# olsonanl/signature_kmers

Measured on AMD Instinct MI355X. Metric: k-mers/sec (extract+hash+count) at 1/2/4/8 GPUs; achieved HBM GB/s %, higher is better.
Workload: dtype u8

## Files before the change

### signature_kmers_amd/__init__.py

```python
from __future__ import annotations

import ctypes as C
import os
from dataclasses import dataclass

import numpy as np

__all__ = [
    "SkmError", "lib", "K", "UNDEFINED_FUNCTION", "STORED_DTYPE", "CALL_DTYPE",
    "SignatureBuilder", "KeptKmers", "CmphKmerDb", "FunctionCaller", "mph_build",
    "kmer_to_str", "str_to_kmer", "keys_from_strings", "device_count", "MatrixDistance", "SeqIdMap",
    "matrix_tile_rows",
]

K = 8
UNDEFINED_FUNCTION = 0xFFFF
_HERE = os.path.dirname(os.path.abspath(__file__))
LIB_PATH = os.environ.get("SKM_LIB_PATH") or os.path.join(_HERE, "libskm.so")

STORED_DTYPE = np.dtype([("avg_from_end", "<u2"), ("function_index", "<u2"), ("mean", "<u2"),
                         ("median", "<u2"), ("var", "<u2")])
CALL_DTYPE = np.dtype([("start", "<u4"), ("end", "<u4"), ("count", "<i4"), ("function_index", "<u2"),
                       ("pad", "<u2"), ("protein_length_median", "<u4"),
                       ("protein_length_med_avg_dev", "<f4")])
# ... 269 lines not shown
            return {}
        ms = (C.c_float * n)()
        cnt = (C.c_uint64 * n)()
        buf = C.create_string_buffer(64 * n + 64)
        lib().skm_build_kernel_timings(self._h, buf, len(buf), ms, cnt, n)
        names = buf.value.decode().split("\n")[:n]
        return {names[i]: (float(ms[i]), int(cnt[i])) for i in range(n)}

    def set_option(self, name: str, value: int):
        _check(lib().skm_build_set_option(self._h, name.encode(), int(value)))

    def passes(self) -> int:
        return self.counters()["passes"]

    def counters(self) -> dict:
        v = (C.c_uint64 * 46)()
        n = lib().skm_build_counters(self._h, v, 46)
        names = ["windows", "kept", "overflow_subbuckets", "chain_jobs", "chain_samples", "sequences", "grouped",
                 "overflow_elements", "overflow_kept", "big_groups", "big_kept", "passes", "valid", "giant_chains",
                 "giant_max", "redone", "cap_overflow_scratch", "cap_split", "cap_long_samples", "cap_long_jobs",
                 "demand_overflow_scratch", "demand_split", "demand_long_samples", "demand_long_jobs",
                 "long_samples", "routed", "add_batch_us", "prepare_upload_us", "prepare_plan_us", "prepare_rest_us",
                 "pass_groups", "add_pack_us", "add_dma_wait_us", "finish_us", "finish_wait_us", "finish_copy_us",
                 "finish_chunks", "finish_select_dev_us", "finish_sort_dev_us", "finish_gather_dev_us",
                 "finish_d2h_dev_us", "finish_max_chunk", "finish_wide_index", "kept_cap",
                 "free_after_prepare", "recs_rot"]
        return {names[i]: int(v[i]) for i in range(n)}

    def debug_jobs(self, k: int = 64) -> list:
        v = (C.c_uint32 * k)()
        _check(lib().skm_build_debug_jobs(self._h, v, k))
        return [int(x) for x in v]

    def debug_overflow(self, k: int = 4096) -> list:
        v = (C.c_uint32 * k)()
        n = lib().skm_build_debug_overflow(self._h, v, k)
        return [int(x) for x in v[:min(max(n, 0), k)]]

    def debug_stamps(self, enable: bool) -> list:
        v = (C.c_uint64 * 32)()
        _check(lib().skm_build_debug_stamps(self._h, 1 if enable else 0, v, 32))
# ... 465 lines not shown
```

### signature_kmers_amd/csrc/skm_build.hip

```cpp
#include <hip/hip_runtime.h>

#include <algorithm>
#include <type_traits>
#include <chrono>
#include <cmath>
#include <cstdio>
#include <cstdlib>
#include <cstring>
#include <deque>
#include <functional>
#include <memory>
#include <numeric>
#include <string>
#include <thread>
#include <vector>

#include "skm_common.h"
#include "skm_pool.h"
#include "skm_output.h"
#include "skm_util.h"

#if defined(SKM_WITH_RCCL)
#include <rccl/rccl.h>
#endif
// ... 616 lines not shown
    return true;
}

enum : uint32_t {
    RUN_FLAGS = 0,
    RUN_LONG_CUR = 1,
    RUN_LONG_N = 2,
    RUN_LONG_FLUSHED = 3,
    RUN_SNAP = 28,
    RUN_DEM_TOT = 8,
    RUN_DEM_SPLIT = 9,
    RUN_DEM_LONG = 10,
    RUN_DEM_LJOBS = 11,
    RUN_LONG_WANT = 12,
    RUN_LONG_WANTJ = 13,
    RUN_ACC_NOVF = 16,
    RUN_ACC_JOBS = 17,
    RUN_ACC_LENS = 18,
    RUN_ACC_OVF_ELEMS = 19,
    RUN_ACC_OVF_KEPT = 20,
    RUN_ACC_BIG = 21,
    RUN_ACC_BIG_KEPT = 22,
    RUN_ACC_GROUPED = 23,
    RUN_LAST_NOVF = 24,
    RUN_LAST_JOBS = 25,
    RUN_NLOC = 26,
    RUN_SLOTS = 64
};
constexpr unsigned long long RUN_F_ARENA = 1;
constexpr unsigned long long RUN_F_RERUN = 2;
constexpr unsigned long long RUN_F_CAP = 4;
enum : uint32_t {
    PLAN_NOVF = 0,
    PLAN_NSPLIT = 1,
    PLAN_NHEAVY = 2,
    PLAN_SKIP = 3,
    PLAN_Q_SPLIT = 4,
    PLAN_Q_HEAVY = 5,
    PLAN_Q_REST = 6,
    PLAN_SLOTS = 8
};

constexpr int JOB_CLASSES = 32;
constexpr int JOB_WG = 256;

__device__ __forceinline__ uint32_t job_class(uint32_t n) { return 31u - (uint32_t)__clz(n | 1u); }

__device__ __forceinline__ void job_chunk(const unsigned long long* nj_p, uint64_t cap, uint64_t& a, uint64_t& e) {
    const uint64_t nj = min((uint64_t)*nj_p, cap);
    const uint64_t chunk = (nj + gridDim.x - 1) / gridDim.x;
    a = min(nj, (uint64_t)blockIdx.x * chunk);
    e = min(nj, a + chunk);
}

// ... 1533 lines not shown
    uint32_t nbuckets;
    uint32_t bucket_base;
    int rem_bits;
    const uint32_t* glen;
    uint8_t* flags;
    unsigned long long* ctr;
    uint64_t* out_keys;
    skm_stored_kmer_data* out_data;
    Job* jobs;
    uint32_t* lens;
    OvfEntry* ovf;
    uint32_t ovf_cap;
    unsigned long long* stamps;
    uint64_t* big_desc;
    uint32_t big_cap;
    int prio;
    int pshift;
    int flag_check;
    const uint32_t* skip;
    uint32_t sub_target;
    int diag;
    const uint32_t* order;
    int part_class;
};

#define SKM_STAMP(i)                                                          \
    do {                                                                      \
        if (A.stamps && threadIdx.x == 0) {                                   \
            const uint64_t _t = __builtin_amdgcn_s_memtime();                 \
            atomicAdd(&A.stamps[(i)], (unsigned long long)(_t - *L.tlast));   \
// ... 186 lines not shown

constexpr uint32_t LPER = CAP / BPK_THREADS;

__device__ __forceinline__ void load_batch(const uint64_t* __restrict__ src_hi, const uint64_t* __restrict__ src_lo,
                                           uint32_t n, uint64_t (&eh)[LPER], uint64_t (&el)[LPER]) {
#pragma unroll
    for (uint32_t u = 0; u < LPER; ++u) {
        const uint32_t j = threadIdx.x + u * BPK_THREADS;
        if (j < n) {
            eh[u] = __builtin_nontemporal_load(src_hi + j);
            el[u] = __builtin_nontemporal_load(src_lo + j);
        }
    }
}

__device__ __forceinline__ void process_sub(const uint64_t* __restrict__ src_hi, const uint64_t* __restrict__ src_lo,
                                            uint32_t n, const BucketArgs& A, uint64_t hprefix, const SubLds& L) {
    const uint32_t tid = threadIdx.x, nt = blockDim.x;
    const uint32_t EMPTY = 0xFFFFFFFFu;
    uint64_t eh[LPER], el[LPER];
    load_batch(src_hi, src_lo, n, eh, el);
    for (uint32_t t = tid; t < (uint32_t)TAB; t += nt) L.tab[t] = EMPTY;
#pragma unroll
    for (uint32_t u = 0; u < LPER; ++u) {
        const uint32_t j = tid + u * BPK_THREADS;
        if (j < n) {
            L.hi[j] = eh[u];
            L.lo[j] = el[u];
        }
    }
    if (tid == 0) *L.nbig = 0;
// ... 78 lines not shown
    if (tid == 0) {
        uint32_t run = 0, acc = 0;
        for (int q = 0; q < 7; ++q) {
            const uint32_t t = ccnt[q];
            ccnt[q] = run;
            cstart[q] = run;
            tstart[q] = acc;
            const uint32_t per = q < 6 ? (64u >> (q + 1)) : 1u;
            acc += (t + per - 1) / per;
            run += t;
        }
        cstart[7] = run;
        tstart[7] = acc;
    }
    unsigned long long big_base = 0;
    if (tid == 0 && cstart[7] > cstart[6]) big_base = atomicAdd(&A.ctr[5], (unsigned long long)(cstart[7] - cstart[6]));
    __syncthreads();
    for (uint32_t g = tid; g < G; g += nt) {
        const uint32_t a = L.goff[L.glist[g]];
        const uint32_t c = g + 1 < G ? L.goff[L.glist[g + 1]] - a : M - a;
        L.big[atomicAdd(&ccnt[cls_of(c)], 1u)] = (uint16_t)g;
    }
    if (tid == 0) *reinterpret_cast<unsigned long long*>(L.wave + 44) = big_base;
    __syncthreads();
    SKM_STAMP(6);
    {
        const uint32_t ntask = tstart[6];
        const uint32_t nbig = cstart[7] - cstart[6];
        const uint64_t bbase = *reinterpret_cast<const unsigned long long*>(L.wave + 44);
        const uint32_t wave = tid >> 6, nwaves = nt >> 6, lane = tid & 63u;
        uint64_t* slots = reinterpret_cast<uint64_t*>(L.lens32);
// ... 91 lines not shown
        }
        const uint64_t jbase = njob ? s_base[1] : 0;
#pragma unroll 1
        for (uint32_t t = tid; t < njob; t += nt) {
            const uint32_t j = L.order[t];
            const uint32_t jb = jobinfo[j];
            Job jbr;
            jbr.lens_off = L.lens_sel + 2 * (jb >> 16);
            jbr.n = jb & JOB_COUNT_MASK;
            jbr.out_idx = (uint32_t)(ob + L.rank[j]);
            A.jobs[jbase + t] = jbr;
        }
    }
    __syncthreads();
    SKM_STAMP(8);
}

__global__ __launch_bounds__(BPK_THREADS, BPK_WAVES_EU) void k_bucket_process(BucketArgs A) {
    static_assert(CAP % BPK_THREADS == 0, "emit assigns CAP / BPK_THREADS elements per thread");
    __shared__ uint64_t s_hi[CAP];
    __shared__ uint64_t s_lo[CAP];
    __shared__ uint32_t s_tab[TAB];
    __shared__ uint32_t s_sub[(1 << MAX_B2) + 1];
    __align__(16) __shared__ uint16_t s_slot[CAP];
    __align__(16) __shared__ uint16_t s_rank[CAP];
    __align__(16) __shared__ uint16_t s_goff[CAP];
    __align__(16) __shared__ uint16_t s_glist[CAP];
    __align__(16) __shared__ uint16_t s_order[CAP];
    __align__(16) __shared__ uint16_t s_big[CAP / 2];
    __shared__ __align__(16) uint32_t s_wave[48];
    __shared__ uint32_t s_nbig;
    __shared__ uint64_t s_tlast;
    __shared__ uint32_t s_ccnt[24];
    if (A.skip && *A.skip) return;
    SubLds L;
    L.ccnt = s_ccnt;
    L.tlast = &s_tlast;
    if (threadIdx.x == 0) s_tlast = __builtin_amdgcn_s_memtime();
    L.hi = s_hi;
    L.lo = s_lo;
    L.tab = s_tab;
    L.slot = s_slot;
    L.rank = s_rank;
    L.goff = s_goff;
    L.glist = s_glist;
    L.order = s_order;
    L.big = s_big;
    L.wave = s_wave;
    L.nbig = &s_nbig;

    const uint32_t bucket = blockIdx.x;
    if (bucket >= A.nbuckets) return;
    const uint64_t r0 = A.bstart[bucket], r1 = A.bstart[bucket + 1];
    const uint64_t n = r1 - r0;
    if (n == 0) return;
    const uint64_t hprefix = (uint64_t)(A.bucket_base + bucket) << A.rem_bits;
    if (A.prio == 1) __builtin_amdgcn_s_setprio(1);
    if (A.prio == 2) __builtin_amdgcn_s_setprio(2);
    if (A.prio >= 3) __builtin_amdgcn_s_setprio(3);

    const bool direct = n <= (uint64_t)CAP && A.nsrc == 1;
    uint32_t nsub = 1;
    if (!direct) {
        const uint32_t* tab = A.sub_tab + (uint64_t)bucket * SUB_TAB;
// ... 472 lines not shown
__global__ __launch_bounds__(BP_THREADS) void k_overflow(BucketArgs A, OvfScratch S, uint32_t* plan, int lo_slot,
                                                          int hi_slot, int q_slot, uint32_t inline_min, int prio) {
    __shared__ uint64_t s_hi[CAP];
    __shared__ uint64_t s_lo[CAP];
    __shared__ __align__(16) uint32_t s_wave[48];
    __shared__ uint32_t s_nbig;
    __shared__ uint32_t s_big[BP_THREADS];
    __shared__ uint32_t s_ninl;
    __shared__ uint64_t s_inl[OVF_INLINE_CAP][2];
    __shared__ uint32_t s_q;
    const uint32_t q_lo = lo_slot < 0 ? 0u : plan[lo_slot], q_hi = plan[hi_slot];
    auto entry = [&](const OvfEntry e) {
        if (e.n == 0) return;
        if ((A.diag & 32) && e.n <= (uint32_t)CAP) return;
        if ((A.diag & 64) && e.n > (uint32_t)CAP) return;
        const uint64_t* src_hi = (e.src == 2 ? S.hi : e.src ? A.tmp_hi : A.recs_hi) + e.off;
        const uint64_t* src_lo = (e.src == 2 ? S.lo : e.src ? A.tmp_lo : A.recs_lo) + e.off;
        uint64_t* ghi = S.hi + e.scratch;
        uint64_t* glo = S.lo + e.scratch;
        uint32_t* heads = S.heads + e.scratch;
        uint64_t* jobinfo = S.jobinfo + e.scratch;
        uint32_t* fmean = S.fmean + e.scratch;
        const uint32_t n = e.n;
        uint32_t N = CAP;
        while (N < n) N <<= 1;
        const uint32_t tid = threadIdx.x, nt = blockDim.x;
        const uint64_t hprefix = (uint64_t)(A.bucket_base + e.bucket) << A.rem_bits;
        const uint32_t nch = (n + CAP - 1) / CAP * CAP;
        for (uint32_t c0 = nch; c0 < N; c0 += CAP)
            for (uint32_t j = tid; j < CAP; j += nt) {
                ghi[c0 + j] = ~0ull;
                glo[c0 + j] = ~0ull;
// ... 216 lines not shown
        }
        __syncthreads();
        const uint32_t q = s_q;
        if (q >= q_hi) break;
        entry(A.ovf[q]);
        __syncthreads();
    }
}

constexpr uint32_t HEAVY_MIN = 1024;
constexpr uint32_t SPLIT_MIN = CAP + 1;
constexpr uint32_t SPLIT_TAB = 4096;
constexpr uint32_t SPLIT_MAXH = 256;
constexpr uint32_t HEAVY_WG = 512;
constexpr uint32_t HEAVY_GRID = 1024;

struct HeavyKey {
    uint64_t off;
    uint32_t n;
    uint32_t bucket;
    uint32_t rem;
    uint32_t pad;
};

struct HeavyArgs {
    HeavyKey* keys;
    unsigned long long* nkeys;
    unsigned long long* cursor;
    unsigned long long* queue;
    uint64_t* rec;
// ... 10 lines not shown
    uint64_t gcap;
    unsigned long long* gstat;
};

__device__ __forceinline__ uint32_t split_hash(uint32_t rem) { return (rem * 0x9E3779B1u) >> (32 - 12); }

__device__ __forceinline__ uint64_t heavy_rec(uint64_t hi, uint64_t lo) {
    return (lo & ~((1ull << 36) - 1ull)) | ((lo & 0xFFFFull) << 16) | (hi & 0xFFFFull);
}
__device__ __forceinline__ uint32_t hr_func(uint64_t x) { return (uint32_t)x & 0xFFFFu; }
__device__ __forceinline__ uint32_t hr_off(uint64_t x) { return (uint32_t)(x >> 16) & 0xFFFFu; }
__device__ __forceinline__ uint32_t hr_seq(uint64_t x) { return (uint32_t)(x >> 36); }

constexpr uint32_t SPLIT_U = 8;

__global__ __launch_bounds__(BP_THREADS) void k_ovf_split(BucketArgs A, OvfScratch S, HeavyArgs H, uint32_t heavy_min,
                                                           uint32_t* plan) {
    static_assert(SPLIT_TAB == 4096, "split_hash yields 12 bits");
    __shared__ uint32_t s_key[SPLIT_TAB];
    __shared__ uint32_t s_cnt[SPLIT_TAB];
    __shared__ uint16_t s_hid[SPLIT_TAB];
    __shared__ uint64_t s_hbase[SPLIT_MAXH];
    __shared__ uint32_t s_hcur[SPLIT_MAXH];
    __shared__ uint32_t s_nh, s_fail, s_lcur, s_heavy;
    const uint32_t tid = threadIdx.x, nt = blockDim.x, lane = tid & 63u;
    __shared__ uint32_t s_q;
    const uint32_t q_hi = plan[PLAN_NSPLIT];
    auto entry = [&](const uint32_t qe) {
        OvfEntry e = A.ovf[qe];
        const uint64_t* src_hi = (e.src ? A.tmp_hi : A.recs_hi) + e.off;
        const uint64_t* src_lo = (e.src ? A.tmp_lo : A.recs_lo) + e.off;
// ... 55 lines not shown
                    const uint64_t hk = atomicAdd(H.nkeys, 1ull);
                    const uint64_t base = atomicAdd(H.cursor, (unsigned long long)s_cnt[q]);
                    s_hbase[h] = base;
                    HeavyKey K;
                    K.off = base;
                    K.n = s_cnt[q];
                    K.bucket = e.bucket;
                    K.rem = s_key[q];
                    K.pad = 0;
                    H.keys[hk] = K;
                    atomicAdd(&s_heavy, s_cnt[q]);
                }
            }
        __syncthreads();
        if (s_heavy == 0) return;
        uint64_t* lhi = S.hi + e.scratch;
        uint64_t* llo = S.lo + e.scratch;
        for (uint32_t j0 = 0; j0 < n; j0 += nt * SPLIT_U) {
            uint64_t eh[SPLIT_U], el[SPLIT_U];
    #pragma unroll
            for (uint32_t u = 0; u < SPLIT_U; ++u) {
                const uint32_t j = j0 + u * nt + tid;
                eh[u] = j < n ? src_hi[j] : ~0ull;
                el[u] = j < n ? src_lo[j] : 0ull;
            }
    #pragma unroll
            for (uint32_t u = 0; u < SPLIT_U; ++u) {
                const bool v = eh[u] != ~0ull;
                uint32_t hid = 0xFFFFu;
                if (v) {
                    const uint32_t rem = (uint32_t)(eh[u] >> 16) & REM_MASK;
                    uint32_t slot = split_hash(rem);
                    while (s_key[slot] != rem) slot = (slot + 1) & (SPLIT_TAB - 1);
                    hid = s_hid[slot];
                }
                const uint64_t lm = __ballot(v && hid == 0xFFFFu);
                uint32_t lbase = 0;
                if (lm) {
                    const uint32_t leader = (uint32_t)(__ffsll((long long)lm) - 1);
                    if (lane == leader) lbase = atomicAdd(&s_lcur, (uint32_t)__popcll(lm));
                    lbase = (uint32_t)__shfl((int)lbase, (int)leader, 64);
                }
                if (v && hid == 0xFFFFu) {
                    const uint32_t pos = lbase + (uint32_t)__popcll(lm & lt);
                    lhi[pos] = eh[u];
                    llo[pos] = el[u];
                }
                const uint32_t h0 = (uint32_t)__builtin_amdgcn_readfirstlane((int)(v ? hid : 0xFFFFu));
                const uint64_t hm = __ballot(v && hid != 0xFFFFu && hid == h0);
                uint32_t hbase = 0;
// ... 1 lines not shown
                    const uint32_t leader = (uint32_t)(__ffsll((long long)hm) - 1);
                    if (lane == leader) hbase = atomicAdd(&s_hcur[h0], (uint32_t)__popcll(hm));
                    hbase = (uint32_t)__shfl((int)hbase, (int)leader, 64);
                }
                if (v && hid != 0xFFFFu) {
                    const uint32_t pos = hid == h0 ? hbase + (uint32_t)__popcll(hm & lt) : atomicAdd(&s_hcur[hid], 1u);
                    const uint64_t o = s_hbase[hid] + pos;
                    H.rec[o] = heavy_rec(eh[u], el[u]);
                    H.len[o] = elem_len(eh[u], el[u], A.glen);
                }
            }
        }
        __syncthreads();
        if (tid == 0) {
            e.n = n - s_heavy;
            e.src = 2;
            e.off = e.scratch;
            A.ovf[qe] = e;
        }
    };
    for (;;) {
        if (tid == 0) s_q = atomicAdd(&plan[PLAN_Q_SPLIT], 1u);
        __syncthreads();
        const uint32_t q = s_q;
        if (q >= q_hi) break;
        entry(q);
        __syncthreads();
    }
}

constexpr int RB = 9;
constexpr uint32_t RBINS = 1u << RB;
__device__ uint32_t* wg_radix_sort_u32(uint32_t* a, uint32_t* b, uint32_t n, int bits, uint32_t* s_hist,
                                       uint32_t (*s_wc)[RBINS], uint32_t* s_run, uint32_t& tag) {
    const uint32_t tid = threadIdx.x, nt = blockDim.x, lane = tid & 63u, wave = tid >> 6, nw = nt >> 6;
    const uint64_t lt = (1ull << lane) - 1ull;
    for (int shift = 0; shift < bits; shift += RB) {
        for (uint32_t d = tid; d < RBINS; d += nt) s_hist[d] = 0;
        __syncthreads();
        for (uint32_t j0 = 0; j0 < n; j0 += nt * SPLIT_U) {
            uint32_t x[SPLIT_U];
#pragma unroll
// ... 585 lines not shown
        const uint64_t tot = s_tot, split = s_split, nl = *P.nloc;
        atomicMax(&R[RUN_DEM_TOT], (unsigned long long)tot);
        atomicMax(&R[RUN_DEM_SPLIT], (unsigned long long)split);
        if (raw > P.ovf_cap) atomicOr(&R[RUN_FLAGS], RUN_F_CAP);
        const bool over = tot > P.tot_cap || split > P.split_cap;
        if (over) atomicOr(&R[RUN_FLAGS], RUN_F_RERUN);
        if (P.kept[0] + nl > P.kept_cap) atomicOr(&R[RUN_FLAGS], RUN_F_ARENA);
        const bool skip = over || (atomicAdd(&R[RUN_FLAGS], 0ull) & (RUN_F_ARENA | RUN_F_CAP)) != 0;
        P.plan[PLAN_NOVF] = skip ? 0u : n;
        P.plan[PLAN_NSPLIT] = skip ? 0u : s_nsplit;
        P.plan[PLAN_NHEAVY] = skip ? 0u : s_nheavy;
        P.plan[PLAN_SKIP] = skip ? 1u : 0u;
        P.plan[PLAN_Q_SPLIT] = 0;
        P.plan[PLAN_Q_HEAVY] = 0;
        P.plan[PLAN_Q_REST] = 0;
        R[RUN_ACC_NOVF] += n;
        R[RUN_ACC_OVF_ELEMS] += s_elems;
        R[RUN_ACC_GROUPED] += nl;
        R[RUN_LAST_NOVF] = n;
    }
}

__global__ void k_poison_jobs(Job* __restrict__ jobs, uint64_t n, uint64_t samples, uint32_t idx,
                             skm_stored_kmer_data* __restrict__ out) {
    const uint64_t t = (uint64_t)blockIdx.x * blockDim.x + threadIdx.x;
    for (uint64_t j = t; j < n; j += (uint64_t)gridDim.x * blockDim.x) jobs[j] = Job{samples, 8u, idx};
    if (t == 0) out[idx] = skm_stored_kmer_data{0xC0DE, 0xC0DE, 0xC0DE, 0xC0DE, 0xC0DE};
}

__global__ void k_pass_account(const unsigned long long* __restrict__ ctr, unsigned long long* __restrict__ run,
                               uint64_t jobs_cap, uint64_t jobs2_cap, uint64_t big_cap, uint64_t lens_cap) {
    const unsigned long long j = ctr[3] + ctr[8 + 3];
    run[RUN_ACC_JOBS] += j;
    run[RUN_ACC_LENS] += ctr[8 + 4];
    run[RUN_ACC_OVF_KEPT] += ctr[8];
    run[RUN_ACC_BIG] += ctr[5];
    run[RUN_ACC_BIG_KEPT] += ctr[6];
    run[RUN_LAST_JOBS] = j;
    if (ctr[3] > jobs_cap || ctr[8 + 3] > jobs2_cap || ctr[5] > big_cap || ctr[8 + 4] > lens_cap)
        atomicOr(&run[RUN_FLAGS], RUN_F_CAP);
}

__global__ void k_kept_finalize(uint64_t* __restrict__ keys, const skm_stored_kmer_data* __restrict__ data,
                                const unsigned long long* __restrict__ n_p, uint32_t nf, uint32_t* __restrict__ dfunc) {
    extern __shared__ uint32_t s_h[];
    const uint64_t n = *n_p;
    const bool lds = nf <= 16384;
    if (lds)
        for (uint32_t f = threadIdx.x; f < nf; f += blockDim.x) s_h[f] = 0;
    __syncthreads();
    for (uint64_t i = (uint64_t)blockIdx.x * blockDim.x + threadIdx.x; i < n; i += (uint64_t)gridDim.x * blockDim.x) {
        keys[i] = decode_key(unmix43(keys[i]));
// ... 126 lines not shown
struct Tune {
    int passes = 0;
    int64_t mem_budget_mb = 0;
    int ovf_heavy = 8192;
    int ovf_inline_min = 0x7FFFFFFF;
    int inline_prio = 3;
    int ovf_long_class = 14;
    int main_long_class = 14;
    int ovf_chain_wgs = 0;
    int chain_prio = 0;
    int bucket_prio = 0;
    int chain_lds_kb = 0;
    int host_timing = 0;
    int heavy_min = (int)HEAVY_MIN;
    int split_min = (int)SPLIT_MIN;
    int giant_class = -1;
    int giant_passes = 0;
    int prefetch = 1;
    int heavy_grid = (int)HEAVY_GRID;
    int ovf_grid = 1024;
    int split_grid = 512;
    int chain_grid = 4096;
    int stream_prio = 0;
    int chain_batches = 2;
    int chain_streams = 1;
    int poison_jobs = 0;
    int route_vacate = 0;
    int tail_async = 1;
    int big_grid = 2048;
    int big_grid_large = 512;
// ... 34 lines not shown
    DevBuf hist, offs, sorted, long_off;
};

struct skm_build {
    skm_build_opts opts{};
    int device = 0;
    hipStream_t stream = nullptr;
    struct EvSet {
        hipEvent_t ev[13] = {}, o[3] = {}, o3[3] = {};
    };
    std::deque<EvSet> evsets;
    hipEvent_t* ev = nullptr;
    hipEvent_t* ev_o = nullptr;
    hipEvent_t* ev_o3 = nullptr;
    float last_ms[15] = {};
    uint64_t ovf_elems = 0, ovf_kept = 0;

    uint8_t* st_pin[2] = {};
    size_t st_fill[2] = {};
    hipEvent_t st_ev[2] = {};
    bool st_busy[2] = {};
    int st_cur = 0;
    uint64_t rp_total = 0;
    uint64_t rp_dev = 0;
    uint64_t res_cap = 0;
    std::vector<SeqMeta> h_meta;
    std::vector<uint32_t> h_seqid;
    std::unique_ptr<HostPool> pool;
    HandoffStats handoff;
    std::vector<uint32_t> h_keep;
    std::vector<uint64_t> h_cum;
// ... 42 lines not shown
#if defined(SKM_WITH_RCCL)
    ncclComm_t comm = nullptr;
#endif
    std::vector<skm_build*> group;
    skm_transport tp{};

    hipStream_t stream2 = nullptr, stream3 = nullptr;
    hipStream_t stream_tail = nullptr;
    hipStream_t stream_tail2 = nullptr;
    hipEvent_t ev_tail_bp = nullptr, ev_tail_done = nullptr, ev_tail2 = nullptr;
    bool tail_pending = false;
    std::function<void()> tail_issue;
    hipEvent_t ev_scan = nullptr;
    bool rot = false;
    uint64_t free_after_prepare = 0;
    hipEvent_t ev_part = nullptr, ev_split = nullptr, ev_part_heavy = nullptr;
    DevBuf d_hv_keys, d_hv_rec, d_hv_len, d_hv_s0, d_hv_s1;
    DevBuf d_sub_tab, d_jobs2, d_jobs3;

    unsigned long long* h_pin = nullptr;
    OvfEntry* h_ovf = nullptr;
    size_t h_ovf_cap = 0;
    unsigned long long* pinned_ctr() {
        if (!h_pin) SKM_HIP(hipHostMalloc(reinterpret_cast<void**>(&h_pin), 128 * 8, hipHostMallocDefault));
        return h_pin;
    }
    OvfEntry* pinned_ovf(size_t n) {
        if (n > h_ovf_cap) {
            if (h_ovf) SKM_HIP(hipHostFree(h_ovf));
            h_ovf = nullptr;
            h_ovf_cap = std::max<size_t>(n, 1024);
// ... 1235 lines not shown
    A.flags = (b->tune.diag & 1) ? nullptr
              : b->tune.flag_bits ? reinterpret_cast<uint8_t*>(reinterpret_cast<uintptr_t>(b->d_flagbits.p) | 1u)
                                  : b->d_flags.as<uint8_t>();
    A.flag_check = b->tune.flag_bits ? 0 : b->tune.flag_check;
    A.ctr = ctr_d;
    A.out_keys = b->d_keys.as<uint64_t>();
    A.out_data = b->d_data.as<skm_stored_kmer_data>();
    A.jobs = b->d_jobs.as<Job>();
    A.lens = b->d_lens.as<uint32_t>();
    A.ovf = b->d_ovf.as<OvfEntry>();
    A.ovf_cap = (uint32_t)b->ovf_cap;
    A.prio = b->tune.bucket_prio;
    A.stamps = nullptr;
    A.big_desc = b->d_big_desc.as<uint64_t>();
    A.big_cap = (uint32_t)std::min<uint64_t>(b->big_cap, 0xFFFFFFFFull);
    A.skip = nullptr;
    A.sub_target = (uint32_t)std::max(0, b->tune.sub_target);
    A.diag = b->tune.diag;
    if (b->stamps) {
        SKM_HIP(hipMemsetAsync(b->d_stamps.p, 0, 32 * 8, st));
        A.stamps = b->d_stamps.as<unsigned long long>();
    }
    A.order = nullptr;
    A.part_class = 0;
    if (b->tune.part_order) {
        b->d_part_order.ensure(4ull * (NB1 + 1));
        SKM_LAUNCH(b, k_part_order, dim3(1), dim3(1024), 0, st, A.bstart, NB1, b->d_part_order.as<uint32_t>());
        A.order = b->d_part_order.as<uint32_t>();
    }
    if (A.order && b->tune.part_split && b->tune.partition_round == 0 && !b->overlap) {
// ... 75 lines not shown
    const bool late = b->tune.giant_passes <= 0 || pass + (uint32_t)b->tune.giant_passes >= NP;
    const int gcls = giant_class(b);
    H.giant_min = gcls > 0 && late && pass < b->gsamples.size() ? 1u << gcls : 0u;
    H.gsamples = nullptr;
    H.gjobs = nullptr;
    H.gcount = nullptr;
    H.gcap = 0;
    H.gstat = nullptr;
    if (H.giant_min) {
        H.gsamples = b->gsamples[pass].as<uint32_t>();
        H.gjobs = b->gjobs[pass].as<Job>();
        H.gcount = b->gcount[pass].as<unsigned long long>();
        H.gcap = giant_cap(b);
        H.gstat = b->d_gstat.as<unsigned long long>();
    }
    auto launch_overflow = [&]() {
    SKM_HIP(hipEventRecord(b->ev_part, st));
    SKM_HIP(hipStreamWaitEvent(st2, b->ev_part, 0));
    SKM_HIP(hipStreamWaitEvent(st3, b->ev_part, 0));
    SKM_HIP(hipEventRecord(b->ev_o[0], st2));
    SKM_HIP(hipEventRecord(b->ev_o3[0], st3));
    if (H.giant_min) SKM_HIP(hipMemsetAsync(b->gcount[pass].p, 0, 16, st2));
    SKM_LAUNCH(b, k_ovf_split, dim3((uint32_t)std::max(1, b->tune.split_grid)), dim3(BP_THREADS), 0, st2, A2, S, H, key_min, plan_d);
    SKM_HIP(hipEventRecord(b->ev_split, st2));
    SKM_HIP(hipStreamWaitEvent(st3, b->ev_split, 0));
    SKM_LAUNCH(b, k_heavy, dim3((uint32_t)std::max(1, b->tune.heavy_grid)), dim3(HEAVY_WG), 0, st2, A2, H);
    SKM_HIP(hipGetLastError());
    if (H.giant_min) {
        SKM_HIP(hipEventRecord(b->gev_ready[gs], st2));
        SKM_HIP(hipStreamWaitEvent(b->gst[gs], b->gev_ready[gs], 0));
        SKM_LAUNCH(b, k_giant_order, dim3(1), dim3(1024), 0, b->gst[gs], H.gjobs, H.gcount);
        if (!b->giant_timed) SKM_HIP(hipEventRecord(b->ev_giant[0], b->gst[gs]));
        SKM_LAUNCH(b, k_chain_dyn, dim3(1024), dim3(128), 0, b->gst[gs], H.gjobs, H.gcount, A.out_data,
                           b->tune.chain_prio);
        SKM_HIP(hipGetLastError());
        if (!b->giant_timed) SKM_HIP(hipEventRecord(b->ev_giant[1], b->gst[gs]));
        b->giant_timed = true;
        SKM_HIP(hipEventRecord(b->gev_done[gs], b->gst[gs]));
        b->gused[gs] = true;
    }
    SKM_LAUNCH(b, k_overflow, dim3((uint32_t)std::max(1, b->tune.ovf_grid)), dim3(BP_THREADS), 0, st2, A2, S, plan_d, -1, (int)PLAN_NHEAVY,
                       (int)PLAN_Q_HEAVY, inline_min, prio);
    SKM_HIP(hipEventRecord(b->ev_o[1], st2));
    SKM_LAUNCH(b, k_overflow, dim3((uint32_t)std::max(1, b->tune.ovf_grid)), dim3(BP_THREADS), 0, st3, A3, S, plan_d, (int)PLAN_NHEAVY,
                       (int)PLAN_NOVF, (int)PLAN_Q_REST, inline_min, prio);
    SKM_HIP(hipGetLastError());
    };
    if (!b->tune.serial_overflow) launch_overflow();
    BigArgs BA;
    BA.desc = A.big_desc;
    BA.ndesc = ctr_d + 5;
    BA.cap = A.big_cap;
    BA.recs_hi = A.recs_hi;
    BA.tmp_hi = A.tmp_hi;
    BA.recs_lo = A.recs_lo;
// ... 6 lines not shown
    SKM_HIP(hipEventRecord(b->ev[5], st));
    if (b->tune.serial_overflow) launch_overflow();
    if (b->pass_bits && pass + 1 < NP && (pass + 1) % b->emit_g == 0 && b->tune.prefetch) {
        SKM_HIP(hipStreamWaitEvent(b->stx, b->ev_staged, 0));
        emit_group(b, (pass + 1) / b->emit_g, b->stx);
        b->emit_q = (pass + 1) / b->emit_g;
    }
    const bool tail_async = tail_async_on(b);
    hipStream_t tt = tail_async ? b->stream_tail : st;
    if (tail_async) {
        SKM_HIP(hipEventRecord(b->ev_tail_bp, st));
        SKM_HIP(hipStreamWaitEvent(tt, b->ev_tail_bp, 0));
    }
    hipEvent_t* ev = b->ev;
    auto big_tail = [=]() {
    if (tail_async && b->tune.big_split) {
        SKM_HIP(hipStreamWaitEvent(b->stream_tail2, b->ev_tail_bp, 0));
        SKM_LAUNCH(b, k_big_groups<true>, dim3((uint32_t)std::max(1, b->tune.big_grid_large)), dim3(BIG_WG), 0,
                   b->stream_tail2, BA);
        SKM_HIP(hipEventRecord(b->ev_tail2, b->stream_tail2));
        SKM_LAUNCH(b, k_big_groups<false>, dim3((uint32_t)std::max(1, b->tune.big_grid)), dim3(BIG_WG), 0, tt, BA);
        SKM_HIP(hipStreamWaitEvent(tt, b->ev_tail2, 0));
    } else {
        SKM_LAUNCH(b, k_big_groups<false>, dim3((uint32_t)std::max(1, b->tune.big_grid)), dim3(BIG_WG), 0, tt, BA);
        SKM_LAUNCH(b, k_big_groups<true>, dim3((uint32_t)std::max(1, b->tune.big_grid_large)), dim3(BIG_WG), 0, tt, BA);
    }
    SKM_LAUNCH(b, k_big_append, dim3(256), dim3(BIG_WG), 0, tt, BA.out, BA, A);
    SKM_HIP(hipGetLastError());
    SKM_HIP(hipEventRecord(ev[12], tt));
    };
    SKM_HIP(hipEventRecord(b->ev_o3[0], st3));
    SKM_HIP(hipStreamWaitEvent(st2, b->ev_o3[0], 0));
    launch_chains(b, st2, A2.jobs, ctr_d + 8 + 3, b->jobs2_cap, b->cs_ovf, A2.lens, nullptr, nullptr, nullptr,
                  A.out_data, (uint32_t)b->tune.ovf_long_class, st3, b->ev_o3[2], (uint32_t)b->tune.ovf_chain_wgs);
    SKM_HIP(hipEventRecord(b->ev_o[2], st2));
    SKM_HIP(hipEventRecord(b->ev_o3[1], st3));
    hipEvent_t* ev_o = b->ev_o;
    hipEvent_t* ev_o3 = b->ev_o3;
    auto main_tail = [=]() {
    big_tail();
    launch_chains(b, tt, A.jobs, ctr_d + 3, b->jobs_cap, b->cs_main, A.lens, reinterpret_cast<const uint32_t*>(A.recs_hi),
                  reinterpret_cast<const uint32_t*>(A.tmp_hi), nullptr, A.out_data, (uint32_t)b->tune.main_long_class);
    if (b->overlap) {
        SKM_HIP(hipEventRecord(b->ev_main_done[ks], st));
        SKM_HIP(hipEventRecord(ev[6], st));
        SKM_HIP(hipStreamWaitEvent(st2, ev_o3[1], 0));
        SKM_HIP(hipStreamWaitEvent(st2, b->ev_main_done[ks], 0));
        SKM_LAUNCH(b, k_pass_account, dim3(1), dim3(1), 0, st2, ctr_d, run_d, b->jobs_cap, b->jobs2_cap, b->big_cap,
                   b->lens_cap);
// ... 262 lines not shown
    if (b->giant_timed) {
        SKM_HIP(hipEventElapsedTime(&b->last_ms[13], b->ev_start, b->ev_giant[0]));
        SKM_HIP(hipEventElapsedTime(&b->last_ms[14], b->ev_start, b->ev_giant[1]));
    }
    b->long_samples = R[RUN_LONG_CUR];
    kt_collect(b);
    b->n_overflow = (uint32_t)R[RUN_ACC_NOVF];
    b->n_overflow_last = (uint32_t)R[RUN_LAST_NOVF];
    b->n_jobs = R[RUN_ACC_JOBS];
    b->n_jobs_last = R[RUN_LAST_JOBS];
    b->n_lens = R[RUN_ACC_LENS];
    b->ovf_elems = R[RUN_ACC_OVF_ELEMS];
    b->ovf_kept = R[RUN_ACC_OVF_KEPT];
    b->n_big = R[RUN_ACC_BIG];
    b->big_kept = R[RUN_ACC_BIG_KEPT];
    b->n_local = R[RUN_ACC_GROUPED];
    b->ran = true;
}

void grow_caps(skm_build* b) {
    auto grow = [](uint64_t& cap, uint64_t dem) {
        if (dem > cap) cap = dem + dem / 8 + 1024;
    };
    grow(b->tot_cap, b->demand[0]);
    grow(b->split_cap, b->demand[1]);
    grow(b->long_cap, b->demand[2]);
    grow(b->long_jobs_cap, b->demand[3]);
    SKM_HIP(hipDeviceSynchronize());
    alloc_caps(b);
}
// ... 113 lines not shown
    }
    for (auto& e : b->chain_ev) SKM_HIP(hipEventCreateWithFlags(&e, hipEventDisableTiming));
    SKM_HIP(hipEventCreateWithFlags(&b->ev_part, hipEventDisableTiming));
    SKM_HIP(hipEventCreateWithFlags(&b->ev_part_heavy, hipEventDisableTiming));
    for (int k = 0; k < 2; ++k) {
        SKM_HIP(hipEventCreateWithFlags(&b->ev_ovf_done[k], hipEventDisableTiming));
        SKM_HIP(hipEventCreateWithFlags(&b->ev_main_done[k], hipEventDisableTiming));
    }
    for (auto& e : b->ev_tail) SKM_HIP(hipEventCreate(&e));
    for (auto& e : b->ev_giant) SKM_HIP(hipEventCreate(&e));
    for (int i = 0; i < 2; ++i) {
        SKM_HIP(hipHostMalloc(reinterpret_cast<void**>(&b->st_pin[i]), STAGE_BYTES, hipHostMallocDefault));
        SKM_HIP(hipEventCreateWithFlags(&b->st_ev[i], hipEventDisableTiming));
    }
    SKM_HIP(hipEventCreateWithFlags(&b->ev_split, hipEventDisableTiming));
    set_geometry(b);
    *out = b;
    SKM_API_END
}

int skm_build_add_batch(skm_build* b, const uint8_t* residues, const uint64_t* seq_off, const uint32_t* seq_len,
                        const uint16_t* seq_func, const uint32_t* seq_id, size_t n_seqs) {
    SKM_API_BEGIN
    SKM_CHECK(b, SKM_E_ARG, "null build");
    SKM_CHECK(n_seqs == 0 || (residues && seq_off && seq_len && seq_func), SKM_E_ARG, "null array");
    SKM_HIP(hipSetDevice(b->device));
    const auto t0 = std::chrono::steady_clock::now();
    std::vector<uint32_t>& ks = b->h_keep;
    ks.clear();
    for (size_t s = 0; s < n_seqs; ++s) {
// ... 291 lines not shown
        SKM_CHECK(value >= 0, SKM_E_ARG, "device_memory_budget_mb must be >= 0");
        t.mem_budget_mb = value;
    } else {
        int* f = n == "overflow_heavy_min" ? &t.ovf_heavy
               : n == "overflow_inline_min" ? &t.ovf_inline_min
               : n == "overflow_inline_prio" ? &t.inline_prio
               : n == "overflow_long_class" ? &t.ovf_long_class
               : n == "main_long_class" ? &t.main_long_class
               : n == "overflow_chain_wgs" ? &t.ovf_chain_wgs
               : n == "chain_prio" ? &t.chain_prio
               : n == "bucket_prio" ? &t.bucket_prio
               : n == "chain_lds_kb" ? &t.chain_lds_kb
               : n == "host_timing" ? &t.host_timing
               : n == "heavy_min" ? &t.heavy_min
               : n == "split_min" ? &t.split_min
               : n == "giant_class" ? &t.giant_class
               : n == "giant_passes" ? &t.giant_passes
               : n == "heavy_lsd" ? &t.heavy_lsd
               : n == "prefetch" ? &t.prefetch
               : n == "overflow_grid" ? &t.ovf_grid
               : n == "split_grid" ? &t.split_grid
               : n == "chain_grid" ? &t.chain_grid
               : n == "chain_batches" ? &t.chain_batches
               : n == "chain_streams" ? &t.chain_streams
               : n == "poison_jobs" ? &t.poison_jobs
               : n == "route_heavy_min" ? &t.route_heavy_min
               : n == "stage_round" ? &t.stage_round
               : n == "partition_round" ? &t.partition_round
               : n == "flag_check" ? &t.flag_check
               : n == "diag" ? &t.diag
// ... 139 lines not shown
    SKM_API_BEGIN
    SKM_CHECK(mismatches && nm, SKM_E_ARG, "bad argument");
    DevBuf d;
    d.ensure(8);
    SKM_HIP(hipMemset(d.p, 0, 8));
    hipLaunchKernelGGL(k_div_check, dim3((uint32_t)ceil_div(nm, 256)), dim3(256), 0, 0, nm, per,
                       d.as<unsigned long long>());
    SKM_HIP(hipGetLastError());
    SKM_HIP(hipMemcpy(mismatches, d.p, 8, hipMemcpyDeviceToHost));
    SKM_API_END
}

int skm_build_counters(skm_build* b, uint64_t* out, int cap) {
    if (!b || !out) return SKM_E_ARG;
    auto us = [](double sec) { return (uint64_t)(sec * 1e6); };
    const uint64_t v[46] = {b->n_windows, b->n_kept, b->n_overflow, b->n_jobs, b->n_lens, b->nseq, b->n_local,
                            b->ovf_elems, b->ovf_kept, b->n_big, b->big_kept, 1ull << b->pass_bits, b->valid_total,
                            b->giant_jobs, b->giant_max, b->n_redo, b->tot_cap, b->split_cap, b->long_cap,
                            b->long_jobs_cap, b->demand[0], b->demand[1], b->demand[2], b->demand[3],
                            b->long_samples, b->routed, us(b->add_s), us(b->prep_upload_s), us(b->prep_plan_s),
                            us(b->prep_rest_s), b->pass_bits ? (1ull << b->pass_bits) / b->emit_g : 0ull, us(b->add_pack_s),
                            us(b->add_wait_s), us(b->handoff.total_s), us(b->handoff.wait_s),
                            us(b->handoff.copy_s), b->handoff.chunks, (uint64_t)(1e3 * b->handoff.select_ms),
                            (uint64_t)(1e3 * b->handoff.sort_ms), (uint64_t)(1e3 * b->handoff.gather_ms),
                            (uint64_t)(1e3 * b->handoff.d2h_ms), b->handoff.max_chunk,
                            (uint64_t)b->handoff.wide_index, b->kept_cap, b->free_after_prepare,
                            (uint64_t)b->rot};
    int n = std::min(cap, 46);
    for (int i = 0; i < n; ++i) out[i] = v[i];
    return n;
}

int skm_build_set_kernel_timing(skm_build* b, int enable, const char* only) {
    SKM_API_BEGIN
    SKM_CHECK(b, SKM_E_ARG, "null build");
    b->kt_mode = enable ? 1 : 0;
    b->kt_only = only ? std::string(only) : std::string();
    SKM_API_END
}

int skm_build_kernel_timings(skm_build* b, char* names, size_t names_cap, float* ms, uint64_t* launches, int cap) {
    if (!b) return SKM_E_ARG;
    const int n = (int)b->kt_names.size();
// ... 242 lines not shown
    for (int k = 0; k < 2; ++k) {
        if (b->ev_ovf_done[k]) (void)hipEventDestroy(b->ev_ovf_done[k]);
        if (b->ev_main_done[k]) (void)hipEventDestroy(b->ev_main_done[k]);
    }
    for (auto& e : b->ev_tail)
        if (e) (void)hipEventDestroy(e);
    for (auto& e : b->ev_giant)
        if (e) (void)hipEventDestroy(e);
    for (auto& e : b->kt_pool) (void)hipEventDestroy(e);
    for (int i = 0; i < 2; ++i) {
        if (b->st_busy[i] && b->st_ev[i]) (void)hipEventSynchronize(b->st_ev[i]);
        if (b->st_pin[i]) (void)hipHostFree(b->st_pin[i]);
        if (b->st_ev[i]) (void)hipEventDestroy(b->st_ev[i]);
    }
    if (b->ev_split) (void)hipEventDestroy(b->ev_split);
    if (b->ev_start) (void)hipEventDestroy(b->ev_start);
    for (int g = 0; g < skm_build::GSLOTS; ++g) {
        if (b->gst[g]) {
            (void)hipStreamSynchronize(b->gst[g]);
            (void)hipStreamDestroy(b->gst[g]);
        }
        if (b->gev_ready[g]) (void)hipEventDestroy(b->gev_ready[g]);
        if (b->gev_done[g]) (void)hipEventDestroy(b->gev_done[g]);
    }
    if (b->stx) {
        (void)hipStreamSynchronize(b->stx);
        (void)hipStreamDestroy(b->stx);
    }
    if (b->ev_staged) (void)hipEventDestroy(b->ev_staged);
    if (b->ev_emit) (void)hipEventDestroy(b->ev_emit);
// ... 29 lines not shown
```

Measured before the change: 11.24 billion.

## Route light overflow sub-buckets through a shared-memory kernel on a side stream

Adds a k_ovf_light kernel that runs on stream st3 after the split. It takes overflow entries that fit in CAP and processes them with the same LDS-based process_sub path as the main bucket kernel, so they no longer go through the generic overflow and chain path. The split kernel now compacts the light remainder in place in the source buffers instead of copying it to scratch, which removes a scratch copy. The change adds cross-stream event dependencies and an in-place write with a __syncthreads to avoid read/write hazards. It also adds counters for the light path.

```diff
diff --git a/signature_kmers_amd/__init__.py b/signature_kmers_amd/__init__.py
--- a/signature_kmers_amd/__init__.py
+++ b/signature_kmers_amd/__init__.py
@@ -307,8 +307,8 @@
         return self.counters()["passes"]
 
     def counters(self) -> dict:
-        v = (C.c_uint64 * 46)()
-        n = lib().skm_build_counters(self._h, v, 46)
+        v = (C.c_uint64 * 48)()
+        n = lib().skm_build_counters(self._h, v, 48)
         names = ["windows", "kept", "overflow_subbuckets", "chain_jobs", "chain_samples", "sequences", "grouped",
                  "overflow_elements", "overflow_kept", "big_groups", "big_kept", "passes", "valid", "giant_chains",
                  "giant_max", "redone", "cap_overflow_scratch", "cap_split", "cap_long_samples", "cap_long_jobs",
@@ -317,7 +317,7 @@
                  "pass_groups", "add_pack_us", "add_dma_wait_us", "finish_us", "finish_wait_us", "finish_copy_us",
                  "finish_chunks", "finish_select_dev_us", "finish_sort_dev_us", "finish_gather_dev_us",
                  "finish_d2h_dev_us", "finish_max_chunk", "finish_wide_index", "kept_cap",
-                 "free_after_prepare", "recs_rot"]
+                 "free_after_prepare", "recs_rot", "overflow_light_subbuckets", "overflow_light_elements"]
         return {names[i]: int(v[i]) for i in range(n)}
 
     def debug_jobs(self, k: int = 64) -> list:
diff --git a/signature_kmers_amd/csrc/skm_build.hip b/signature_kmers_amd/csrc/skm_build.hip
--- a/signature_kmers_amd/csrc/skm_build.hip
+++ b/signature_kmers_amd/csrc/skm_build.hip
@@ -654,6 +654,8 @@
     RUN_DEM_LJOBS = 11,
     RUN_LONG_WANT = 12,
     RUN_LONG_WANTJ = 13,
+    RUN_ACC_LIGHT_SUB = 14,
+    RUN_ACC_LIGHT_ELEMS = 15,
     RUN_ACC_NOVF = 16,
     RUN_ACC_JOBS = 17,
     RUN_ACC_LENS = 18,
@@ -678,6 +680,7 @@
     PLAN_Q_SPLIT = 4,
     PLAN_Q_HEAVY = 5,
     PLAN_Q_REST = 6,
+    PLAN_Q_LIGHT = 7,
     PLAN_SLOTS = 8
 };
 
@@ -2241,6 +2244,7 @@
     unsigned long long* stamps;
     uint64_t* big_desc;
     uint32_t big_cap;
+    unsigned long long* big_ctr;
     int prio;
     int pshift;
     int flag_check;
@@ -2457,7 +2461,7 @@
     }
 }
 
-__device__ __forceinline__ void process_sub(const uint64_t* __restrict__ src_hi, const uint64_t* __restrict__ src_lo,
+__device__ __forceinline__ uint32_t process_sub(const uint64_t* __restrict__ src_hi, const uint64_t* __restrict__ src_lo,
                                             uint32_t n, const BucketArgs& A, uint64_t hprefix, const SubLds& L) {
     const uint32_t tid = threadIdx.x, nt = blockDim.x;
     const uint32_t EMPTY = 0xFFFFFFFFu;
@@ -2566,7 +2570,7 @@
         tstart[7] = acc;
     }
     unsigned long long big_base = 0;
-    if (tid == 0 && cstart[7] > cstart[6]) big_base = atomicAdd(&A.ctr[5], (unsigned long long)(cstart[7] - cstart[6]));
+    if (tid == 0 && cstart[7] > cstart[6]) big_base = atomicAdd(A.big_ctr, (unsigned long long)(cstart[7] - cstart[6]));
     __syncthreads();
     for (uint32_t g = tid; g < G; g += nt) {
         const uint32_t a = L.goff[L.glist[g]];
@@ -2688,40 +2692,52 @@
     }
     __syncthreads();
     SKM_STAMP(8);
+    return nkept;
+}
+
+struct SubMem {
+    uint64_t hi[CAP];
+    uint64_t lo[CAP];
+    uint32_t tab[TAB];
+    __align__(16) uint16_t slot[CAP];
+    __align__(16) uint16_t rank[CAP];
+    __align__(16) uint16_t goff[CAP];
+    __align__(16) uint16_t glist[CAP];
+    __align__(16) uint16_t order[CAP];
+    __align__(16) uint16_t big[CAP / 2];
+    __align__(16) uint32_t wave[48];
+    uint32_t nbig;
+    uint64_t tlast;
+    uint32_t ccnt[24];
+};
+
+__device__ __forceinline__ SubLds sub_lds(SubMem& m) {
+    SubLds L;
+    L.ccnt = m.ccnt;
+    L.tlast = &m.tlast;
+    if (threadIdx.x == 0) m.tlast = __builtin_amdgcn_s_memtime();
+    L.hi = m.hi;
+    L.lo = m.lo;
+    L.tab = m.tab;
+    L.slot = m.slot;
+    L.rank = m.rank;
+    L.goff = m.goff;
+    L.glist = m.glist;
+    L.order = m.order;
+    L.big = m.big;
+    L.wave = m.wave;
+    L.nbig = &m.nbig;
+    L.lens32 = nullptr;
+    L.lens_sel = 0;
+    return L;
 }
 
 __global__ __launch_bounds__(BPK_THREADS, BPK_WAVES_EU) void k_bucket_process(BucketArgs A) {
     static_assert(CAP % BPK_THREADS == 0, "emit assigns CAP / BPK_THREADS elements per thread");
-    __shared__ uint64_t s_hi[CAP];
-    __shared__ uint64_t s_lo[CAP];
-    __shared__ uint32_t s_tab[TAB];
+    __shared__ SubMem s_mem;
     __shared__ uint32_t s_sub[(1 << MAX_B2) + 1];
-    __align__(16) __shared__ uint16_t s_slot[CAP];
-    __align__(16) __shared__ uint16_t s_rank[CAP];
-    __align__(16) __shared__ uint16_t s_goff[CAP];
-    __align__(16) __shared__ uint16_t s_glist[CAP];
-    __align__(16) __shared__ uint16_t s_order[CAP];
-    __align__(16) __shared__ uint16_t s_big[CAP / 2];
-    __shared__ __align__(16) uint32_t s_wave[48];
-    __shared__ uint32_t s_nbig;
-    __shared__ uint64_t s_tlast;
-    __shared__ uint32_t s_ccnt[24];
     if (A.skip && *A.skip) return;
-    SubLds L;
-    L.ccnt = s_ccnt;
-    L.tlast = &s_tlast;
-    if (threadIdx.x == 0) s_tlast = __builtin_amdgcn_s_memtime();
-    L.hi = s_hi;
-    L.lo = s_lo;
-    L.tab = s_tab;
-    L.slot = s_slot;
-    L.rank = s_rank;
-    L.goff = s_goff;
-    L.glist = s_glist;
-    L.order = s_order;
-    L.big = s_big;
-    L.wave = s_wave;
-    L.nbig = &s_nbig;
+    SubLds L = sub_lds(s_mem);
 
     const uint32_t bucket = blockIdx.x;
     if (bucket >= A.nbuckets) return;
@@ -3224,8 +3240,8 @@
         if (e.n == 0) return;
         if ((A.diag & 32) && e.n <= (uint32_t)CAP) return;
         if ((A.diag & 64) && e.n > (uint32_t)CAP) return;
-        const uint64_t* src_hi = (e.src == 2 ? S.hi : e.src ? A.tmp_hi : A.recs_hi) + e.off;
-        const uint64_t* src_lo = (e.src == 2 ? S.lo : e.src ? A.tmp_lo : A.recs_lo) + e.off;
+        const uint64_t* src_hi = (e.src ? A.tmp_hi : A.recs_hi) + e.off;
+        const uint64_t* src_lo = (e.src ? A.tmp_lo : A.recs_lo) + e.off;
         uint64_t* ghi = S.hi + e.scratch;
         uint64_t* glo = S.lo + e.scratch;
         uint32_t* heads = S.heads + e.scratch;
@@ -3472,6 +3488,7 @@
 constexpr uint32_t SPLIT_MAXH = 256;
 constexpr uint32_t HEAVY_WG = 512;
 constexpr uint32_t HEAVY_GRID = 1024;
+constexpr uint32_t LIGHT_GRID = 128;
 
 struct HeavyKey {
     uint64_t off;
@@ -3512,7 +3529,7 @@
 
 constexpr uint32_t SPLIT_U = 8;
 
-__global__ __launch_bounds__(BP_THREADS) void k_ovf_split(BucketArgs A, OvfScratch S, HeavyArgs H, uint32_t heavy_min,
+__global__ __launch_bounds__(BP_THREADS) void k_ovf_split(BucketArgs A, HeavyArgs H, uint32_t heavy_min,
                                                            uint32_t* plan) {
     static_assert(SPLIT_TAB == 4096, "split_hash yields 12 bits");
     __shared__ uint32_t s_key[SPLIT_TAB];
@@ -3598,10 +3615,11 @@
             }
         __syncthreads();
         if (s_heavy == 0) return;
-        uint64_t* lhi = S.hi + e.scratch;
-        uint64_t* llo = S.lo + e.scratch;
+        uint64_t* lhi = const_cast<uint64_t*>(src_hi);
+        uint64_t* llo = const_cast<uint64_t*>(src_lo);
         for (uint32_t j0 = 0; j0 < n; j0 += nt * SPLIT_U) {
             uint64_t eh[SPLIT_U], el[SPLIT_U];
+            uint32_t hids[SPLIT_U];
     #pragma unroll
             for (uint32_t u = 0; u < SPLIT_U; ++u) {
                 const uint32_t j = j0 + u * nt + tid;
@@ -3610,14 +3628,20 @@
             }
     #pragma unroll
             for (uint32_t u = 0; u < SPLIT_U; ++u) {
-                const bool v = eh[u] != ~0ull;
-                uint32_t hid = 0xFFFFu;
-                if (v) {
+                hids[u] = 0xFFFFu;
+                if (eh[u] != ~0ull) {
                     const uint32_t rem = (uint32_t)(eh[u] >> 16) & REM_MASK;
                     uint32_t slot = split_hash(rem);
                     while (s_key[slot] != rem) slot = (slot + 1) & (SPLIT_TAB - 1);
-                    hid = s_hid[slot];
+                    hids[u] = s_hid[slot];
                 }
+                asm volatile("" : "+v"(el[u]));
+            }
+            __syncthreads();
+    #pragma unroll
+            for (uint32_t u = 0; u < SPLIT_U; ++u) {
+                const bool v = eh[u] != ~0ull;
+                const uint32_t hid = hids[u];
                 const uint64_t lm = __ballot(v && hid == 0xFFFFu);
                 uint32_t lbase = 0;
                 if (lm) {
@@ -3649,8 +3673,6 @@
         __syncthreads();
         if (tid == 0) {
             e.n = n - s_heavy;
-            e.src = 2;
-            e.off = e.scratch;
             A.ovf[qe] = e;
         }
     };
@@ -3661,6 +3683,39 @@
         if (q >= q_hi) break;
         entry(q);
         __syncthreads();
+    }
+}
+
+__global__ __launch_bounds__(BPK_THREADS, BPK_WAVES_EU) void k_ovf_light(BucketArgs A, uint32_t* plan,
+                                                                         unsigned long long* stat) {
+    __shared__ SubMem s_mem;
+    __shared__ uint32_t s_q;
+    if (A.skip && *A.skip) return;
+    SubLds L = sub_lds(s_mem);
+    const uint32_t q_hi = plan[PLAN_NOVF];
+    unsigned long long kept = 0, nel = 0;
+    uint32_t nsub = 0;
+    for (;;) {
+        if (threadIdx.x == 0) s_q = atomicAdd(&plan[PLAN_Q_LIGHT], 1u);
+        __syncthreads();
+        const uint32_t q = s_q;
+        if (q >= q_hi) break;
+        const OvfEntry e = A.ovf[q];
+        if (e.n != 0 && e.n <= (uint32_t)CAP && e.src == 1) {
+            const uint64_t hprefix = (uint64_t)(A.bucket_base + e.bucket) << A.rem_bits;
+            L.lens_sel = (LENS_IN_TMP << LENS_SEL_SHIFT) | (2 * e.off);
+            L.lens32 = reinterpret_cast<uint32_t*>(A.tmp_hi + e.off);
+            kept += process_sub(A.tmp_hi + e.off, A.tmp_lo + e.off, e.n, A, hprefix, L);
+            if (threadIdx.x == 0) A.ovf[q].n = 0;
+            ++nsub;
+            nel += e.n;
+        }
+        __syncthreads();
+    }
+    if (threadIdx.x == 0 && nsub) {
+        atomicAdd(&A.ctr[0], kept);
+        atomicAdd(&stat[0], (unsigned long long)nsub);
+        atomicAdd(&stat[1], nel);
     }
 }
 
@@ -4276,6 +4331,7 @@
         P.plan[PLAN_Q_SPLIT] = 0;
         P.plan[PLAN_Q_HEAVY] = 0;
         P.plan[PLAN_Q_REST] = 0;
+        P.plan[PLAN_Q_LIGHT] = 0;
         R[RUN_ACC_NOVF] += n;
         R[RUN_ACC_OVF_ELEMS] += s_elems;
         R[RUN_ACC_GROUPED] += nl;
@@ -4298,6 +4354,8 @@
     run[RUN_ACC_OVF_KEPT] += ctr[8];
     run[RUN_ACC_BIG] += ctr[5];
     run[RUN_ACC_BIG_KEPT] += ctr[6];
+    run[RUN_ACC_LIGHT_SUB] += ctr[21];
+    run[RUN_ACC_LIGHT_ELEMS] += ctr[22];
     run[RUN_LAST_JOBS] = j;
     if (ctr[3] > jobs_cap || ctr[8 + 3] > jobs2_cap || ctr[5] > big_cap || ctr[8 + 4] > lens_cap)
         atomicOr(&run[RUN_FLAGS], RUN_F_CAP);
@@ -4454,6 +4512,7 @@
     int host_timing = 0;
     int heavy_min = (int)HEAVY_MIN;
     int split_min = (int)SPLIT_MIN;
+    int ovf_light = 1;
     int giant_class = -1;
     int giant_passes = 0;
     int prefetch = 1;
@@ -4518,7 +4577,7 @@
     hipEvent_t* ev_o = nullptr;
     hipEvent_t* ev_o3 = nullptr;
     float last_ms[15] = {};
-    uint64_t ovf_elems = 0, ovf_kept = 0;
+    uint64_t ovf_elems = 0, ovf_kept = 0, ovf_light_sub = 0, ovf_light_elems = 0;
 
     uint8_t* st_pin[2] = {};
     size_t st_fill[2] = {};
@@ -4591,7 +4650,7 @@
     hipEvent_t ev_scan = nullptr;
     bool rot = false;
     uint64_t free_after_prepare = 0;
-    hipEvent_t ev_part = nullptr, ev_split = nullptr, ev_part_heavy = nullptr;
+    hipEvent_t ev_part = nullptr, ev_split = nullptr, ev_part_heavy = nullptr, ev_light = nullptr;
     DevBuf d_hv_keys, d_hv_rec, d_hv_len, d_hv_s0, d_hv_s1;
     DevBuf d_sub_tab, d_jobs2, d_jobs3;
 
@@ -5857,6 +5916,7 @@
     A.stamps = nullptr;
     A.big_desc = b->d_big_desc.as<uint64_t>();
     A.big_cap = (uint32_t)std::min<uint64_t>(b->big_cap, 0xFFFFFFFFull);
+    A.big_ctr = ctr_d + 5;
     A.skip = nullptr;
     A.sub_target = (uint32_t)std::max(0, b->tune.sub_target);
     A.diag = b->tune.diag;
@@ -5962,6 +6022,7 @@
         H.gcap = giant_cap(b);
         H.gstat = b->d_gstat.as<unsigned long long>();
     }
+    const bool light = b->tune.ovf_light != 0;
     auto launch_overflow = [&]() {
     SKM_HIP(hipEventRecord(b->ev_part, st));
     SKM_HIP(hipStreamWaitEvent(st2, b->ev_part, 0));
@@ -5969,9 +6030,14 @@
     SKM_HIP(hipEventRecord(b->ev_o[0], st2));
     SKM_HIP(hipEventRecord(b->ev_o3[0], st3));
     if (H.giant_min) SKM_HIP(hipMemsetAsync(b->gcount[pass].p, 0, 16, st2));
-    SKM_LAUNCH(b, k_ovf_split, dim3((uint32_t)std::max(1, b->tune.split_grid)), dim3(BP_THREADS), 0, st2, A2, S, H, key_min, plan_d);
+    SKM_LAUNCH(b, k_ovf_split, dim3((uint32_t)std::max(1, b->tune.split_grid)), dim3(BP_THREADS), 0, st2, A2, H, key_min, plan_d);
     SKM_HIP(hipEventRecord(b->ev_split, st2));
     SKM_HIP(hipStreamWaitEvent(st3, b->ev_split, 0));
+    if (light) {
+        SKM_LAUNCH(b, k_ovf_light, dim3(LIGHT_GRID), dim3(BPK_THREADS), 0, st3, A3, plan_d,
+                   ctr_d + 21);
+        SKM_HIP(hipEventRecord(b->ev_light, st3));
+    }
     SKM_LAUNCH(b, k_heavy, dim3((uint32_t)std::max(1, b->tune.heavy_grid)), dim3(HEAVY_WG), 0, st2, A2, H);
     SKM_HIP(hipGetLastError());
     if (H.giant_min) {
@@ -5987,6 +6053,7 @@
         SKM_HIP(hipEventRecord(b->gev_done[gs], b->gst[gs]));
         b->gused[gs] = true;
     }
+    if (light) SKM_HIP(hipStreamWaitEvent(st2, b->ev_light, 0));
     SKM_LAUNCH(b, k_overflow, dim3((uint32_t)std::max(1, b->tune.ovf_grid)), dim3(BP_THREADS), 0, st2, A2, S, plan_d, -1, (int)PLAN_NHEAVY,
                        (int)PLAN_Q_HEAVY, inline_min, prio);
     SKM_HIP(hipEventRecord(b->ev_o[1], st2));
@@ -6023,8 +6090,10 @@
     }
     hipEvent_t* ev = b->ev;
     auto big_tail = [=]() {
+    if (light) SKM_HIP(hipStreamWaitEvent(tt, b->ev_light, 0));
     if (tail_async && b->tune.big_split) {
         SKM_HIP(hipStreamWaitEvent(b->stream_tail2, b->ev_tail_bp, 0));
+        if (light) SKM_HIP(hipStreamWaitEvent(b->stream_tail2, b->ev_light, 0));
         SKM_LAUNCH(b, k_big_groups<true>, dim3((uint32_t)std::max(1, b->tune.big_grid_large)), dim3(BIG_WG), 0,
                    b->stream_tail2, BA);
         SKM_HIP(hipEventRecord(b->ev_tail2, b->stream_tail2));
@@ -6040,8 +6109,8 @@
     };
     SKM_HIP(hipEventRecord(b->ev_o3[0], st3));
     SKM_HIP(hipStreamWaitEvent(st2, b->ev_o3[0], 0));
-    launch_chains(b, st2, A2.jobs, ctr_d + 8 + 3, b->jobs2_cap, b->cs_ovf, A2.lens, nullptr, nullptr, nullptr,
-                  A.out_data, (uint32_t)b->tune.ovf_long_class, st3, b->ev_o3[2], (uint32_t)b->tune.ovf_chain_wgs);
+    launch_chains(b, st2, A2.jobs, ctr_d + 8 + 3, b->jobs2_cap, b->cs_ovf, A2.lens, reinterpret_cast<const uint32_t*>(A.recs_hi),
+                  reinterpret_cast<const uint32_t*>(A.tmp_hi), nullptr, A.out_data, (uint32_t)b->tune.ovf_long_class, st3, b->ev_o3[2], (uint32_t)b->tune.ovf_chain_wgs);
     SKM_HIP(hipEventRecord(b->ev_o[2], st2));
     SKM_HIP(hipEventRecord(b->ev_o3[1], st3));
     hipEvent_t* ev_o = b->ev_o;
@@ -6334,6 +6403,8 @@
     b->ovf_kept = R[RUN_ACC_OVF_KEPT];
     b->n_big = R[RUN_ACC_BIG];
     b->big_kept = R[RUN_ACC_BIG_KEPT];
+    b->ovf_light_sub = R[RUN_ACC_LIGHT_SUB];
+    b->ovf_light_elems = R[RUN_ACC_LIGHT_ELEMS];
     b->n_local = R[RUN_ACC_GROUPED];
     b->ran = true;
 }
@@ -6477,6 +6548,7 @@
         SKM_HIP(hipEventCreateWithFlags(&b->st_ev[i], hipEventDisableTiming));
     }
     SKM_HIP(hipEventCreateWithFlags(&b->ev_split, hipEventDisableTiming));
+    SKM_HIP(hipEventCreateWithFlags(&b->ev_light, hipEventDisableTiming));
     set_geometry(b);
     *out = b;
     SKM_API_END
@@ -6798,6 +6870,7 @@
                : n == "host_timing" ? &t.host_timing
                : n == "heavy_min" ? &t.heavy_min
                : n == "split_min" ? &t.split_min
+               : n == "ovf_light" ? &t.ovf_light
                : n == "giant_class" ? &t.giant_class
                : n == "giant_passes" ? &t.giant_passes
                : n == "heavy_lsd" ? &t.heavy_lsd
@@ -6967,7 +7040,7 @@
 int skm_build_counters(skm_build* b, uint64_t* out, int cap) {
     if (!b || !out) return SKM_E_ARG;
     auto us = [](double sec) { return (uint64_t)(sec * 1e6); };
-    const uint64_t v[46] = {b->n_windows, b->n_kept, b->n_overflow, b->n_jobs, b->n_lens, b->nseq, b->n_local,
+    const uint64_t v[48] = {b->n_windows, b->n_kept, b->n_overflow, b->n_jobs, b->n_lens, b->nseq, b->n_local,
                             b->ovf_elems, b->ovf_kept, b->n_big, b->big_kept, 1ull << b->pass_bits, b->valid_total,
                             b->giant_jobs, b->giant_max, b->n_redo, b->tot_cap, b->split_cap, b->long_cap,
                             b->long_jobs_cap, b->demand[0], b->demand[1], b->demand[2], b->demand[3],
@@ -6978,8 +7051,8 @@
                             (uint64_t)(1e3 * b->handoff.sort_ms), (uint64_t)(1e3 * b->handoff.gather_ms),
                             (uint64_t)(1e3 * b->handoff.d2h_ms), b->handoff.max_chunk,
                             (uint64_t)b->handoff.wide_index, b->kept_cap, b->free_after_prepare,
-                            (uint64_t)b->rot};
-    int n = std::min(cap, 46);
+                            (uint64_t)b->rot, b->ovf_light_sub, b->ovf_light_elems};
+    int n = std::min(cap, 48);
     for (int i = 0; i < n; ++i) out[i] = v[i];
     return n;
 }
@@ -7252,6 +7325,7 @@
         if (b->st_ev[i]) (void)hipEventDestroy(b->st_ev[i]);
     }
     if (b->ev_split) (void)hipEventDestroy(b->ev_split);
+    if (b->ev_light) (void)hipEventDestroy(b->ev_light);
     if (b->ev_start) (void)hipEventDestroy(b->ev_start);
     for (int g = 0; g < skm_build::GSLOTS; ++g) {
         if (b->gst[g]) {
```

After: 11.76 billion (median of 6 runs). 4.6% higher.
